# cordum-io/cordum

Hardware: AMD Instinct MI355X
Metric: jobs dispatched/sec (whole node) (higher is better)
Workload: dtype int64-bitset/int32 (control-plane integer path); 1 GPU; model=cordum control-plane dispatch pipeline (echo workers), global_batch=16384, seq_len=256, parallelism=shard1, rules=1024, workers_per_rank=1000, denied_jobs=14465

## Files before the change

cordum_amd/ops/hip/cordum_kernels.hip:

```cpp
#include <hip/hip_runtime.h>
#include <cstdint>

#define WAVE 64
#define BLOCK 256


template <int W, int JPT>
__global__ __launch_bounds__(BLOCK) void policy_first_match_kernel(
    const long long* __restrict__ rule_any,
    const long long* __restrict__ rule_all,
    const signed char* __restrict__ rule_secrets,
    const long long* __restrict__ rule_mcp,
    const unsigned char* __restrict__ rule_mcp_any,
    const long long* __restrict__ job_any,
    const long long* __restrict__ job_all,
    const unsigned char* __restrict__ job_secrets,
    const long long* __restrict__ job_mcp,
    const unsigned char* __restrict__ job_mcp_used,
    int* __restrict__ out_first,
    int R, int J, int rules_per_chunk)
{
    const int rule_chunk_begin = blockIdx.y * rules_per_chunk;
    const int rule_chunk_end = min(R, rule_chunk_begin + rules_per_chunk);
    constexpr int ANY_W = 7 * W;
// ... 1657 lines not shown
__global__ __launch_bounds__(BLOCK) void policy_first_match_mfma_bits_kernel(
    const long long* __restrict__ any_bits,
    const long long* __restrict__ all_bits,
    const signed char* __restrict__ b_pack,
    const int* __restrict__ cards,
    const signed char* __restrict__ rule_secrets,
    const unsigned char* __restrict__ job_secrets,
    const int* __restrict__ tile_dims,
    int* __restrict__ out_first,
    int J, int R, int tiles_per_chunk)
{
    const int lane = threadIdx.x % WAVE;
    const int shift = (lane >> 4) * 16;
    v4i afrag[TJ][9];
    #pragma unroll
    for (int t = 0; t < TJ; ++t) {
        const int job = (blockIdx.x * TJ + t) * 16 + (lane & 15);
        #pragma unroll
        for (int d = 0; d < 9; ++d) {
            unsigned long long w = 0;
            if (job < J)
                w = (unsigned long long)(d < 7 ? any_bits[(size_t)job * 7 + d]
                                               : all_bits[(size_t)job * 2 + (d - 7)]);
            const unsigned int slice = (unsigned int)(w >> shift) & 0xFFFFu;
            #pragma unroll
            for (int q = 0; q < 4; ++q)
                afrag[t][d][q] = (int)((((slice >> (4 * q)) & 0xFu) * 0x00204081u) & 0x01010101u);
        }
    }
    mfma_first_match_tiles<TJ>(afrag, b_pack, cards, rule_secrets, job_secrets,
                               tile_dims, out_first, J, R, tiles_per_chunk);
}


__global__ __launch_bounds__(BLOCK) void policy_gate_kernel(
    const int* __restrict__ first,
    const signed char* __restrict__ decisions,
    signed char* __restrict__ out_decision,
    int* __restrict__ denied_slots,
    int* __restrict__ denied_count,
    int* __restrict__ allowed_slots,
    int* __restrict__ allowed_count,
    int J, int R)
{
    const int j = blockIdx.x * BLOCK + threadIdx.x;
    const int lane = threadIdx.x % WAVE;
    gate_job(j, J, lane, first, decisions, R, out_decision,
             allowed_slots, allowed_count, denied_slots, denied_count);
}

__global__ __launch_bounds__(BLOCK) void policy_gate_full_kernel(
    const int* __restrict__ first,
    const signed char* __restrict__ decisions,
    signed char* __restrict__ out_decision,
    int* __restrict__ denied_slots,
    int* __restrict__ denied_count,
    int* __restrict__ allowed_slots,
    int* __restrict__ allowed_count,
    unsigned char* __restrict__ states,
    long long* __restrict__ deadlines,
    int* __restrict__ dlq_ring,
    int* __restrict__ dlq_head,
    int ring_size,
    int J, int R)
{
    const int j = blockIdx.x * BLOCK + threadIdx.x;
// ... 894 lines not shown
    torch::Tensor tile_dims, int64_t n_rules, torch::Tensor out, int64_t job_tiles)
{
    CHECK_DEV(any_bits); CHECK_DEV(b_pack);
    CHECK_CONTIG(any_bits); CHECK_CONTIG(all_bits);
    TORCH_CHECK(job_tiles == 1 || job_tiles == 2, "job_tiles must be 1 or 2");
    TORCH_CHECK(any_bits.dim() == 3 && any_bits.size(1) == 7 && any_bits.size(2) == 1 &&
                all_bits.dim() == 3 && all_bits.size(1) == 2 && all_bits.size(2) == 1,
                "MFMA K1 needs the 1-word vocab: any [J,7,1], all [J,2,1]");
    const int J = (int)any_bits.size(0), R = (int)n_rules;
    TORCH_CHECK(all_bits.size(0) == J && job_secrets.size(0) >= J && out.size(0) >= J,
                "job tensors must cover J");
    const int TJ = (int)job_tiles;
    const int Jt = ((J + 15) / 16 + TJ - 1) / TJ;
    const int Rt = (R + 15) / 16;
    if (J == 0 || R == 0) return;
    TORCH_CHECK(b_pack.size(0) >= Rt && tile_dims.size(0) >= Rt &&
                rule_secrets.size(0) >= Rt * 16 && cards.size(0) >= Rt * 16,
                "rule pack smaller than n_rules");
    int nchunks = std::max(1, std::min((Rt + 3) / 4, std::max(1, 2048 / std::max(Jt, 1))));
    const int tiles_per_chunk = (Rt + nchunks - 1) / nchunks;
    auto launch = [&](auto kernel) {
        hipLaunchKernelGGL(kernel, dim3(Jt, nchunks), dim3(BLOCK), 0, cur_stream(),
            (const long long*)any_bits.data_ptr<int64_t>(),
            (const long long*)all_bits.data_ptr<int64_t>(),
            (const signed char*)b_pack.data_ptr<int8_t>(),
            cards.data_ptr<int>(),
            (const signed char*)rule_secrets.data_ptr<int8_t>(),
            job_secrets.data_ptr<uint8_t>(),
            tile_dims.data_ptr<int>(),
            out.data_ptr<int>(), J, R, tiles_per_chunk);
    };
    if (TJ == 2) launch(policy_first_match_mfma_bits_kernel<2>);
    else launch(policy_first_match_mfma_bits_kernel<1>);
}

void gate_route(torch::Tensor first, torch::Tensor decisions, torch::Tensor out_decision,
                torch::Tensor denied_slots, torch::Tensor denied_count,
                torch::Tensor allowed_slots, torch::Tensor allowed_count,
                torch::Tensor states, torch::Tensor deadlines,
                torch::Tensor dlq_ring, torch::Tensor dlq_head,
                torch::Tensor pick, torch::Tensor order, torch::Tensor valid_count,
                torch::Tensor j_poolmask, torch::Tensor j_labels,
                int64_t full_mask, int64_t K,
                torch::Tensor routable_slots, torch::Tensor routable_widx,
                torch::Tensor routable_count, torch::Tensor extra_zero)
{
    CHECK_DEV(first);
    const int J = (int)first.size(0);
    TORCH_CHECK(out_decision.size(0) >= J && denied_slots.size(0) >= J &&
                allowed_slots.size(0) >= J && states.size(0) >= J &&
                deadlines.size(0) >= J && pick.size(0) >= J &&
                j_poolmask.size(0) >= J && j_labels.size(0) >= J &&
                routable_slots.size(0) >= J && routable_widx.size(0) >= J,
                "per-job tensors must cover J");
    TORCH_CHECK(K <= order.size(0), "K exceeds the order table");
    const int n_extra = (int)extra_zero.size(0);
    const int blocks = (std::max(std::max(J, n_extra), 1) + BLOCK - 1) / BLOCK;
    hipLaunchKernelGGL(gate_route_kernel, dim3(blocks), dim3(BLOCK), 0, cur_stream(),
        first.data_ptr<int>(), (const signed char*)decisions.data_ptr<int8_t>(),
        (signed char*)out_decision.data_ptr<int8_t>(),
        denied_slots.data_ptr<int>(), denied_count.data_ptr<int>(),
        allowed_slots.data_ptr<int>(), allowed_count.data_ptr<int>(),
        states.data_ptr<uint8_t>(), (long long*)deadlines.data_ptr<int64_t>(),
        dlq_ring.data_ptr<int>(), dlq_head.data_ptr<int>(), (int)dlq_ring.size(0),
        pick.data_ptr<int>(), order.data_ptr<int>(), valid_count.data_ptr<int>(),
        (const long long*)j_poolmask.data_ptr<int64_t>(),
// ... 660 lines not shown
                             int64_t all_requires,
                             c10::optional<torch::Tensor> payload,
                             int64_t payload_words,
                             int64_t threads, int64_t isa_cap)
{
    TORCH_CHECK(!any_bits.is_cuda() && !all_bits.is_cuda(),
                "synthetic_fresh_stamped is a host encoder");
    CHECK_CONTIG(any_bits); CHECK_CONTIG(all_bits);
    CHECK_CONTIG(tenant_lut); CHECK_CONTIG(topic_lut);
    CHECK_CONTIG(risk_lut); CHECK_CONTIG(req_lut);
    cordum_enc::EncodeJob a;
    a.B = any_bits.size(0);
    a.W = any_bits.size(2);
    a.V = tenant_lut.size(0);
    TORCH_CHECK(any_bits.size(1) == 7 && all_bits.size(0) == a.B &&
                all_bits.size(1) == 2 && all_bits.size(2) == a.W, "bad batch shape");
    for (const torch::Tensor* l : {&tenant_lut, &topic_lut, &risk_lut, &req_lut})
        TORCH_CHECK(l->size(0) == a.V && l->size(1) == a.W, "bad LUT shape");
    TORCH_CHECK(dim_tenant >= 0 && dim_tenant < 7 && dim_topic >= 0 && dim_topic < 7 &&
                dim_risk >= 0 && dim_risk < 7 && all_requires >= 0 && all_requires < 2,
                "dim index out of range");
    a.any = any_bits.data_ptr<int64_t>();
    a.all = all_bits.data_ptr<int64_t>();
    a.tenant_lut = tenant_lut.data_ptr<int64_t>();
    a.topic_lut = topic_lut.data_ptr<int64_t>();
    a.risk_lut = risk_lut.data_ptr<int64_t>();
    a.req_lut = req_lut.data_ptr<int64_t>();
    a.seed = (uint64_t)seed;
    a.step = (uint64_t)step;
    a.dim_tenant = (int)dim_tenant;
    a.dim_topic = (int)dim_topic;
    a.dim_risk = (int)dim_risk;
    a.all_requires = (int)all_requires;
    a.payload = nullptr;
    a.payload_words = payload_words;
    if (payload.has_value()) {
        TORCH_CHECK(!payload->is_cuda() && payload->is_contiguous() &&
                    payload->scalar_type() == torch::kInt32 && payload_words > 0 &&
                    payload->numel() >= a.B * payload_words, "bad payload ring buffer");
        a.payload = payload->data_ptr<int32_t>();
    }
    cordum_enc::encode_batch(a, (int)threads, (int)isa_cap);
}

void pack_jobs_mfma_dev(torch::Tensor any_bits, torch::Tensor all_bits,
                        torch::Tensor a_pack)
{
    const int B = (int)any_bits.size(0);
    const int Jt = (int)a_pack.size(0);
    const int n = Jt * 9 * 64;
    const int blocks = (n + BLOCK - 1) / BLOCK;
    hipLaunchKernelGGL(pack_jobs_mfma_kernel, dim3(blocks), dim3(BLOCK), 0, cur_stream(),
        (const long long*)any_bits.data_ptr<int64_t>(),
        (const long long*)all_bits.data_ptr<int64_t>(),
        a_pack.data_ptr<int8_t>(), B, Jt);
}

PYBIND11_MODULE(TORCH_EXTENSION_NAME, m) {
    m.def("policy_first_match", &policy_first_match, "K1 batched policy first-match");
    m.def("policy_first_match_mfma", &policy_first_match_mfma, "K1 MFMA comparison variant");
    m.def("worker_precompute", &worker_precompute, "K2a per-worker score/overload precompute");
    m.def("least_loaded_pick", &least_loaded_pick, "K2 least-loaded worker pick");
    m.def("spread_pick", &spread_pick, "K2c batch spreading over the least-loaded set");
    m.def("worker_precompute_into", &worker_precompute_into, "K2a into a persistent key tensor");
    m.def("dlq_ring_append", &dlq_ring_append, "K7 device DLQ ring append");
    m.def("echo_execute_indexed", &echo_execute_indexed, "device echo worker pool (slot-indexed, in-place)");
    m.def("policy_gate", &policy_gate, "decision gather + allow/deny compaction");
    m.def("policy_gate_full", &policy_gate_full,
          "gate + DENIED transition + DLQ ring append in one launch");
    m.def("begin_tick", &begin_tick, "tick prologue: PENDING re-admit + counter reset");
    m.def("accumulate_counts", &accumulate_counts, "fold tick counters into device accumulator");
    m.def("begin_tick_first", &begin_tick_first,
          "tick prologue that also primes the first-match buffer (INT_MAX)");
    m.def("least_loaded_pick_into", &least_loaded_pick_into,
          "K2 pick into a persistent buffer, skipping unconstrained jobs");
    m.def("policy_first_match_mfma_into", &policy_first_match_mfma_into,
          "K1 MFMA into a pre-primed buffer (no alloc/fill launches)");
    m.def("compact_routable_spread", &compact_routable_spread,
          "routable compaction with inline K2c spread");
    m.def("apply_transitions_chain_dyn", &apply_transitions_chain_dyn,
          "K5 chained targets in one launch (+ extra zero region)");
    m.def("compact_routable", &compact_routable, "routable-slot compaction");
    m.def("apply_transitions_dyn", &apply_transitions_dyn, "K5 with device-resident count");
    m.def("echo_execute_indexed_dyn", &echo_execute_indexed_dyn, "echo worker with device count");
    m.def("load_feedback", &load_feedback, "per-worker active-count histogram");
    m.def("run_readiness", &run_readiness, "K3 run/step readiness sweep");
    m.def("synthetic_fresh", &synthetic_fresh,
          py::call_guard<py::gil_scoped_release>(),
          "fused host synthetic-batch encoder");
    m.def("pack_jobs_mfma_dev", &pack_jobs_mfma_dev, "device job packing for the MFMA K1");
    m.def("synthetic_fresh_stamped", &synthetic_fresh_stamped,
          py::call_guard<py::gil_scoped_release>(),
          "host batch preparation in one call: synthetic dims + payload step stamp",
          py::arg("any_bits"), py::arg("all_bits"), py::arg("tenant_lut"),
          py::arg("topic_lut"), py::arg("risk_lut"), py::arg("req_lut"),
          py::arg("seed"), py::arg("step"), py::arg("dim_tenant"), py::arg("dim_topic"),
          py::arg("dim_risk"), py::arg("all_requires"), py::arg("payload"),
          py::arg("payload_words"), py::arg("threads") = 1, py::arg("isa_cap") = -1);
    m.def("encoder_isa_level", [] { return cordum_enc::max_isa_level(); },
          "widest encoder ISA this CPU runs (0 baseline, 1 AVX2, 2 AVX-512DQ)");
    m.def("tick_prologue", &tick_prologue,
          "fused tick 1/5: PENDING re-admit + counter reset + first prime + worker keys");
    m.def("policy_first_match_mfma_bits_into", &policy_first_match_mfma_bits_into,
          "fused tick 3/5: K1 MFMA with A fragments built from the staged bit words",
          py::arg("any_bits"), py::arg("all_bits"), py::arg("b_pack"), py::arg("cards"),
          py::arg("rule_secrets"), py::arg("job_secrets"), py::arg("tile_dims"),
          py::arg("n_rules"), py::arg("out"), py::arg("job_tiles") = 1);
    m.def("gate_route", &gate_route,
          "fused tick 4/5: gate + DENIED/DLQ + spread/exact pick + routable compaction");
    m.def("tick_finish", &tick_finish,
          "fused tick 5/5: echo + state chain + load feedback + counter fold");
    m.def("pack_by_dest", &pack_by_dest, "padded per-destination dispatch pack");
    m.def("pack_requeue", &pack_requeue, "redeliver last tick's requeue ring into the send segments");
    m.def("wf_sweep", &wf_sweep, "K3-WF readiness sweep + approval holds + condition/delay commits");
    m.def("wf_expand", &wf_expand, "K3-WF for_each/worker child expansion into the child arena");
    m.def("wf_apply", &wf_apply, "K3-WF child result application with failure injection");
    m.def("wf_apply_dead", &wf_apply_dead, "K3-WF dead-letter child application");
    m.def("wf_commit", &wf_commit, "K3-WF step aggregation + retry/backoff commit");
    m.def("wf_timeout_scan", &wf_timeout_scan, "K4-WF stale-step timeout scan");
    m.def("wf_readmit", &wf_readmit, "K3-WF continuous run re-admission from template");
    m.def("wf_status", &wf_status, "K3-WF run status roll-up");
    m.def("wf_grant", &wf_grant, "K3-WF host approval grants");
    m.def("wf_admit", &wf_admit, "K3-WF run admission into the lowest free slots");
    m.def("wf_cancel", &wf_cancel, "K3-WF generation-checked run cancellation");
    m.def("wf_retire", &wf_retire, "K3-WF completion records + quiescent slot release");
    m.def("wf_journal", &wf_journal, "K3-WF step-transition journal pass (observer)");
    m.def("wf_hold_scan", &wf_hold_scan, "K3-WF approval hold scan (open / expire / close holds)");
    m.def("wf_settle", &wf_settle, "K3-WF per-step-policy timeout + commit pass (replaces the scan/commit pair)");
    m.def("wf_hold_list", &wf_hold_list, "K3-WF ordered page of open approval holds");
    m.def("wf_decide", &wf_decide, "K3-WF generation-checked approval decisions");
    m.def("materialize_rq_payload", &materialize_rq_payload, "copy requeued payload rows into the rq arena");
    m.def("gather_payload_padded", &gather_payload_padded, "payload gather into padded send arena");
    m.def("echo_padded", &echo_padded, "region-valid echo over padded recv arena");
    m.def("apply_transitions_padded", &apply_transitions_padded, "K5 over padded slot list");
    m.def("load_feedback_padded", &load_feedback_padded, "padded per-worker load histogram");
    m.def("set_transition_lut", &set_transition_lut, "upload transition legality LUT");
    m.def("apply_transitions", &apply_transitions, "K5 batched state transitions");
    m.def("deadline_scan", &deadline_scan, "K4 deadline/staleness scan");
// ... 3 lines not shown
```

cordum_amd/ops/hip/synthetic_encode.h:

```cpp
#pragma once

#include <cstddef>
#include <cstdint>
#include <thread>

namespace cordum_enc {

struct EncodeJob {
    int64_t* any;
    int64_t* all;
    const int64_t* tenant_lut;
    const int64_t* topic_lut;
    const int64_t* risk_lut;
    const int64_t* req_lut;
    int64_t B, W, V;
    uint64_t seed, step;
    int dim_tenant, dim_topic, dim_risk, all_requires;
    int32_t* payload;
    int64_t payload_words;
};

constexpr int kBlock = 64;
constexpr uint32_t kRiskCut = 1288490189u;
constexpr uint32_t kReqCut = 429496730u;

static inline uint64_t splitmix64(uint64_t x) {
    x += 0x9E3779B97F4A7C15ull;
    x = (x ^ (x >> 30)) * 0xBF58476D1CE4E5B9ull;
    x = (x ^ (x >> 27)) * 0x94D049BB133111EBull;
    return x ^ (x >> 31);
}

static inline uint64_t batch_base(uint64_t seed, uint64_t step) {
    return splitmix64(seed * 0x5851F42D4C957F2Dull ^ step);
}

__attribute__((always_inline)) static inline void encode_range_impl(
    const EncodeJob& a, int64_t i0, int64_t i1)
{
    const uint64_t base = batch_base(a.seed, a.step);
    const uint64_t v = (uint64_t)a.V;
    const int64_t W = a.W;
    const int32_t stamp = (int32_t)(uint32_t)a.step;
    uint32_t t_idx[kBlock], o_idx[kBlock], r_idx[kBlock], q_idx[kBlock];
    uint32_t c_risk[kBlock], c_req[kBlock];
    for (int64_t b0 = i0; b0 < i1; b0 += kBlock) {
        const int n = (int)((i1 - b0) < kBlock ? (i1 - b0) : kBlock);
        for (int k = 0; k < kBlock; ++k) {
            const uint64_t h0 = splitmix64(base ^ (uint64_t)(b0 + k));
            const uint64_t h1 = splitmix64(h0);
            const uint64_t h2 = splitmix64(h1);
            t_idx[k] = (uint32_t)(((h0 & 0xffffffffull) * v) >> 32);
            o_idx[k] = (uint32_t)(((h0 >> 32) * v) >> 32);
            r_idx[k] = (uint32_t)(((h1 & 0xffffffffull) * v) >> 32);
            q_idx[k] = (uint32_t)(((h1 >> 32) * v) >> 32);
            c_risk[k] = (uint32_t)h2;
            c_req[k] = (uint32_t)(h2 >> 32);
        }
        if (W == 1) {
            int64_t* arow = a.any + (size_t)b0 * 7;
            int64_t* lrow = a.all + (size_t)b0 * 2;
            for (int k = 0; k < n; ++k, arow += 7, lrow += 2) {
                arow[a.dim_tenant] = a.tenant_lut[t_idx[k]];
                arow[a.dim_topic] = a.topic_lut[o_idx[k]];
                arow[a.dim_risk] = c_risk[k] < kRiskCut ? a.risk_lut[r_idx[k]] : 0;
                lrow[a.all_requires] = c_req[k] < kReqCut ? a.req_lut[q_idx[k]] : 0;
            }
        } else {
            for (int k = 0; k < n; ++k) {
                int64_t* arow = a.any + (size_t)(b0 + k) * 7 * W;
                int64_t* lrow = a.all + (size_t)(b0 + k) * 2 * W;
                const bool has_risk = c_risk[k] < kRiskCut;
                const bool has_req = c_req[k] < kReqCut;
                const int64_t* tl = a.tenant_lut + (size_t)t_idx[k] * W;
                const int64_t* ol = a.topic_lut + (size_t)o_idx[k] * W;
                const int64_t* rl = a.risk_lut + (size_t)r_idx[k] * W;
                const int64_t* ql = a.req_lut + (size_t)q_idx[k] * W;
                for (int64_t w = 0; w < W; ++w) {
                    arow[a.dim_tenant * W + w] = tl[w];
                    arow[a.dim_topic * W + w] = ol[w];
                    arow[a.dim_risk * W + w] = has_risk ? rl[w] : 0;
                    lrow[a.all_requires * W + w] = has_req ? ql[w] : 0;
                }
            }
        }
        if (a.payload != nullptr) {
            int32_t* p = a.payload + (size_t)b0 * a.payload_words;
            for (int k = 0; k < n; ++k, p += a.payload_words) *p = stamp;
        }
    }
}

static void encode_range_base(const EncodeJob& a, int64_t i0, int64_t i1) {
    encode_range_impl(a, i0, i1);
}

#if defined(__x86_64__) && (defined(__GNUC__) || defined(__clang__)) && \
    !defined(__HIP_DEVICE_COMPILE__)
#define CORDUM_ENC_MULTIVERSION 1
__attribute__((target("avx2"))) static void encode_range_avx2(
    const EncodeJob& a, int64_t i0, int64_t i1) {
    encode_range_impl(a, i0, i1);
}
__attribute__((target("avx512f,avx512dq,avx512vl"))) static void encode_range_avx512(
    const EncodeJob& a, int64_t i0, int64_t i1) {
    encode_range_impl(a, i0, i1);
}
static inline int max_isa_level() {
    __builtin_cpu_init();
    if (__builtin_cpu_supports("avx512f") && __builtin_cpu_supports("avx512dq") &&
        __builtin_cpu_supports("avx512vl"))
        return 2;
    if (__builtin_cpu_supports("avx2")) return 1;
    return 0;
}
// ... 29 lines not shown
```

cordum_amd/ops/pipeline.py:

```python
from __future__ import annotations

import time
from dataclasses import dataclass
from typing import List, Optional

import torch
import torch.distributed as dist

from ..protocol.states import transition_lut
from ..safety import policy as pol
from . import get_ext
from .policy_compile import CompiledPolicy, JobBatch, JobEncoder, compile_policy, first_match_reference

UNSPECIFIED, PENDING, APPROVAL, SCHEDULED, DISPATCHED, RUNNING = 0, 1, 2, 3, 4, 5
SUCCEEDED, FAILED, CANCELLED, TIMEOUT, DENIED = 6, 7, 8, 9, 10

ALLOW_CODES = (1, 5)


@dataclass
class TickStats:
    completed: int = 0
    denied: int = 0
    unrouted: int = 0
# ... 102 lines not shown
        out.any_bits[:, DIM_TOPIC].copy_(row)
        torch.index_select(self.risk_lut, 0, r_idx, out=row)
        mask.view(-1).copy_(u_risk < 0.3)
        row.mul_(mask)
        out.any_bits[:, DIM_RISK].copy_(row)
        torch.index_select(self.req_lut, 0, q_idx, out=row)
        mask.view(-1).copy_(u_req < 0.1)
        row.mul_(mask)
        out.all_bits[:, ALL_REQUIRES].copy_(row)

    def fresh_fast(self, out: JobBatch, step: int, ext) -> None:
        DIM_TENANT, DIM_TOPIC, DIM_RISK, ALL_REQUIRES = self._dims
        ext.synthetic_fresh(out.any_bits, out.all_bits,
                            self.tenant_lut, self.topic_lut,
                            self.risk_lut, self.req_lut,
                            self.seed, step,
                            DIM_TENANT, DIM_TOPIC, DIM_RISK, ALL_REQUIRES)

    encode_threads = 1

    def fresh_stamped(self, out: JobBatch, step: int, ext, payload: torch.Tensor,
                      payload_words: int, threads: Optional[int] = None,
                      isa_cap: int = -1) -> None:
        DIM_TENANT, DIM_TOPIC, DIM_RISK, ALL_REQUIRES = self._dims
        ext.synthetic_fresh_stamped(out.any_bits, out.all_bits,
                                    self.tenant_lut, self.topic_lut,
                                    self.risk_lut, self.req_lut,
                                    self.seed, step,
                                    DIM_TENANT, DIM_TOPIC, DIM_RISK, ALL_REQUIRES,
                                    payload, payload_words,
                                    self.encode_threads if threads is None else threads,
                                    isa_cap)


class _RefOps:

    def __init__(self):
        self._lut = None

    def set_transition_lut(self, lut):
        self._lut = lut

    def policy_first_match(self, rule_any, rule_all, rule_secrets, rule_mcp, rule_mcp_any,
                           job_any, job_all, job_secrets, job_mcp, job_mcp_used, chunks):
        from types import SimpleNamespace

        c = SimpleNamespace(any_masks=rule_any, all_masks=rule_all, secrets=rule_secrets,
                            mcp_masks=rule_mcp, mcp_any=rule_mcp_any,
                            n_rules=int(rule_any.shape[0]))
        b = SimpleNamespace(any_bits=job_any, all_bits=job_all, secrets=job_secrets,
                            mcp_bits=job_mcp, mcp_used=job_mcp_used,
                            n_jobs=int(job_any.shape[0]))
        return first_match_reference(c, b)

    def worker_precompute(self, w_pool, w_active, w_maxp, w_cpu, w_gpu):
        from .reference import worker_precompute_ref

        return worker_precompute_ref(w_pool, w_active, w_maxp, w_cpu, w_gpu)

    def least_loaded_pick(self, w_pool, w_keys, w_labels, j_poolmask, j_labels):
        from .reference import least_loaded_pick_keys_ref

        return least_loaded_pick_keys_ref(w_pool, w_keys, w_labels, j_poolmask, j_labels)

    def echo_execute_indexed(self, ctx_arena, slots, res_arena, res_sum, stride):
        from .reference import echo_execute_indexed_ref
# ... 275 lines not shown
        return apply_transitions_ref(states, attempts, deadlines, slots, to_states)

    def echo_execute(self, ctx_arena, res_arena, stride):
        from .reference import echo_execute_ref

        return echo_execute_ref(ctx_arena, res_arena, int(stride))


def alloc_batch_staging(B: int, W: int, device=None, pin: bool = False):
    n64 = B * 7 * W + B * 2 * W + B * 4 * W
    nbytes = ((n64 * 8 + 2 * B + 7) // 8) * 8
    if pin:
        buf = torch.zeros(nbytes, dtype=torch.uint8).pin_memory()
    else:
        buf = torch.zeros(nbytes, dtype=torch.uint8, device=device)
    o = 0

    def take64(*shape):
        nonlocal o
        n = 1
        for s in shape:
            n *= s
        t = buf[o:o + n * 8].view(torch.int64).view(*shape)
        o += n * 8
        return t

    any_b = take64(B, 7, W)
    all_b = take64(B, 2, W)
    mcp_b = take64(B, 4, W)
    sec = buf[o:o + B]
    o += B
    used = buf[o:o + B]
    return JobBatch(any_b, all_b, sec, mcp_b, used), buf


def alloc_result_block(B: int, device=None, pin: bool = False):
    nbytes = ((4 * B + 16 + B + 7) // 8) * 8
    if pin:
        buf = torch.zeros(nbytes, dtype=torch.uint8).pin_memory()
    else:
        buf = torch.zeros(nbytes, dtype=torch.uint8, device=device)
    sums = buf[0:4 * B].view(torch.int32)
    counts = buf[4 * B:4 * B + 16].view(torch.int32)
    dec = buf[4 * B + 16:5 * B + 16].view(torch.int8)
    return sums, counts, dec, buf


class DevicePipeline:
    def __init__(
        self,
        device: torch.device,
        batch_size: int = 16384,
        n_local_workers: int = 1000,
        n_rules: int = 1024,
        payload_words: int = 64,
        world_size: int = 1,
        rank: int = 0,
        n_batches: int = 8,
        policy: Optional[pol.SafetyPolicy] = None,
        seed: int = 7,
        backend: str = "ext",
        use_mfma: Optional[bool] = None,
        mfma_pack_on_device: bool = False,
        pad_cap: Optional[int] = None,
        unfused_tick: bool = False,
        k1_job_tiles: int = 2,
    ):
        self._k1_job_tiles = k1_job_tiles
        self._pad_cap_override = pad_cap
        self._unfused_tick = unfused_tick
        self._mfma_device_pack = mfma_pack_on_device
        device = torch.device(device)
        self.ext = _RefOps() if backend == "ref" else get_ext(required=True)
        self.device = device
        self.B = batch_size
        self.NWL = n_local_workers
        self.world = world_size
        self.rank = rank
        self.payload_words = payload_words

        self.ext.set_transition_lut(torch.tensor(transition_lut(), dtype=torch.uint8).flatten())

        policy = policy or make_synthetic_policy(n_rules, seed=seed)
        for w in (1, 2, 4):
            self.compiled = compile_policy(policy, words=w)
            if self.compiled.exact:
                break
        assert self.compiled.exact, "bench policy must compile exactly"
        self.cpol = self.compiled.to(device)

        self.batches: List[JobBatch] = []
        self.batch_bufs: List[torch.Tensor] = []
        self.payloads: List[torch.Tensor] = []
        for i in range(n_batches):
            jb = encode_synthetic_jobs(self.compiled, self.B, seed=seed * 1000 + i + rank * 77)
            dev_jb, dev_buf = alloc_batch_staging(self.B, self.compiled.words,
                                                  device=device)
            dev_jb.any_bits.copy_(jb.any_bits)
            dev_jb.all_bits.copy_(jb.all_bits)
# ... 60 lines not shown
            backend != "ref"
            and device.type == "cuda"
            and world_size == 1
            and self.compiled.words == 1
            and self.compiled.n_rules <= 32768
            and int(self.compiled.mcp_any.sum()) == 0
        )
        if use_mfma is False:
            self._use_mfma = False
        if self._use_mfma and self._mfma_device_pack:
            from .policy_mfma import N_DIMS, pack_policy_mfma

            self.mfma_policy = pack_policy_mfma(self.compiled).to(device)
            self.mfma_a_packs = []
            if self._unfused_tick:
                Jt = (self.B + 15) // 16
                self.mfma_a_packs = [
                    torch.zeros(Jt, N_DIMS, 64, 16, dtype=torch.int8, device=device)
                    for _ in range(len(self.batches))
                ]
        elif self._use_mfma:
            from .policy_mfma import pack_jobs_mfma, pack_policy_mfma

            self.mfma_policy = pack_policy_mfma(self.compiled).to(device)
            self.mfma_a_packs = []
            for jb_host, jb_dev in zip(
                [encode_synthetic_jobs(self.compiled, self.B, seed=seed * 1000 + i + rank * 77)
                 for i in range(len(self.batches) if self._unfused_tick else 0)],
                self.batches
            ):
                a_pack, _ = pack_jobs_mfma(jb_host)
                self.mfma_a_packs.append(a_pack.to(device))
        self._fused_capable = device.type == "cuda" and self.world == 1 and backend != "ref"
        self._tick = 0
        self.total_completed = 0
        self.total_denied = 0


    def _spread(self, pick):
        full_mask = (1 << self.world) - 1
        K = min(int(self.order_buf.shape[0]), 1024)
        self.ext.spread_pick(self.order_buf, self.valid_buf, self.j_poolmask,
                             self.j_labels, full_mask, pick, K)
        return pick

    def _refresh_order(self) -> None:
        if self._tick % 8 != 1:
            return
        self.order_buf.copy_(torch.argsort(self.w_keys).to(torch.int32))
        valid = ((self.w_keys >> 32) & 0xFFFFFFFF).ne(0xFFFFFFFE)
        self.valid_buf.copy_(valid.sum().to(torch.int32).reshape(1))

    def _fused_body(self, slot: int) -> None:
        if self._unfused_tick:
            return self._unfused_body(slot)
        B = self.B
        ext = self.ext
        jb = self.batches[slot]
        full_mask = (1 << self.world) - 1
        ext.tick_prologue(self.states, self._counts,
                          self.first_buf if self._use_mfma else None,
                          self.w_active_local, self.w_maxp,
                          self.w_cpu_local, self.w_gpu_local, self.w_keys)
        ext.least_loaded_pick_into(self.w_pool, self.w_keys, self.w_labels,
                                   self.j_poolmask, self.j_labels,
                                   self.valid_buf, full_mask, self.pick_buf)
        if self._use_mfma:
            ext.policy_first_match_mfma_bits_into(
                jb.any_bits, jb.all_bits, self.mfma_policy.b_pack,
                self.mfma_policy.cards, self.mfma_policy.secrets, jb.secrets,
                self.mfma_policy.tile_dims, self.compiled.n_rules, self.first_buf,
                self._k1_job_tiles)
            first = self.first_buf
        else:
            first = ext.policy_first_match(
                self.cpol.any_masks, self.cpol.all_masks, self.cpol.secrets,
                self.cpol.mcp_masks, self.cpol.mcp_any,
                jb.any_bits, jb.all_bits, jb.secrets, jb.mcp_bits, jb.mcp_used, 0,
            )
        K = min(int(self.order_buf.shape[0]), 1024)
        ext.gate_route(first, self.cpol.decisions, self.out_decision,
                       self.denied_slots, self.denied_count,
                       self.allowed_slots, self.allowed_count,
                       self.states, self.deadlines, self.dlq_ring, self.dlq_head,
                       self.pick_buf, self.order_buf, self.valid_buf,
                       self.j_poolmask, self.j_labels, full_mask, K,
                       self.routable_slots, self.routable_widx,
                       self.routable_count, self.w_active_local)
        ext.tick_finish(self.payloads[slot], self.routable_slots,
                        self.routable_widx, self.routable_count,
                        self.res_arena[: B * self.payload_words], self.res_sums,
                        self.payload_words,
                        self.states, self.attempts, self.deadlines,
                        [SCHEDULED, DISPATCHED, RUNNING, SUCCEEDED],
                        self.w_active_local, self.NWL, self.rank,
                        self._counts, self.acc_counts, B)

    def _unfused_body(self, slot: int) -> None:
        B = self.B
        ext = self.ext
# ... 36 lines not shown
                                    self.routable_count)
        ext.echo_execute_indexed_dyn(self.payloads[slot], self.routable_slots,
                                     self.routable_count, self.res_arena[: B * self.payload_words],
                                     self.res_sums, self.payload_words, B)
        ext.apply_transitions_chain_dyn(self.states, self.attempts, self.deadlines,
                                        self.routable_slots, self.routable_count,
                                        [SCHEDULED, DISPATCHED, RUNNING, SUCCEEDED],
                                        self.w_active_local, B)
        ext.load_feedback(self.routable_widx, self.routable_count,
                          self.w_active_local, self.NWL, self.rank, B)
        ext.accumulate_counts(self._counts, self.acc_counts)

    def _ensure_graphs(self) -> None:
        if self._graphs:
            return
        side = torch.cuda.Stream(device=self.device)
        side.wait_stream(torch.cuda.current_stream(self.device))
        with torch.cuda.stream(side):
            for slot in range(len(self.batches)):
                self._fused_body(slot)
        torch.cuda.current_stream(self.device).wait_stream(side)
        torch.cuda.synchronize(self.device)
        for slot in range(len(self.batches)):
            g = torch.cuda.CUDAGraph()
            with torch.cuda.graph(g):
                self._fused_body(slot)
            self._graphs[slot] = g
        self._graph = self._graphs[0]
        self.dlq_head.zero_()
        self.dlq_ring.fill_(-1)
        self.acc_counts.zero_()
        torch.cuda.synchronize(self.device)

    def _replay_fused(self) -> None:
        i = self._tick % len(self.batches)
        self._tick += 1
        self._graphs[i].replay()
        self._refresh_order()

    def _tick_fused(self) -> TickStats:
        self._ensure_graphs()
        t0 = time.perf_counter()
        self._replay_fused()
        counts = self._counts.cpu()
        denied = int(counts[0])
        routable = int(counts[2])
        dt = time.perf_counter() - t0
        stats = TickStats(
            completed=routable,
            denied=denied,
            unrouted=self.B - routable - denied,
            wall_s=dt,
        )
        self.total_completed += stats.completed
        self.total_denied += stats.denied
        return stats

    def ensure_e2e(self, seed: int = 11, payload_ring: int = 4) -> None:
        if hasattr(self, "_e2e_enc"):
            return
        assert not self._use_mfma or self._mfma_device_pack, \
            "e2e ingest needs staged descriptors: bitset K1 or device-packed MFMA"
        self._e2e_enc = SyntheticEncoder(self.compiled, seed=seed + self.rank)
        pin = self.device.type == "cuda"
        B, W = self.B, self.compiled.words

# ... 109 lines not shown
            return self._e2e_run_dist(steps)
        if self.device.type != "cuda" or not self._fused_capable:
            completed = denied = 0
            lats = []
            for _ in range(steps):
                st = self.tick_e2e()
                completed += st.completed
                denied += st.denied
                lats.append(st.wall_s)
            return completed, denied, lats

        self._ensure_graphs()
        B = self.B
        nslots = 2
        nhost = 4
        if not hasattr(self, "_e2e_hosts2"):
            Wc = self.compiled.words
            pairs = [alloc_batch_staging(B, Wc, pin=True) for _ in range(nhost)]
            self._e2e_hosts2 = [p[0] for p in pairs]
            self._e2e_host_bufs = [p[1] for p in pairs]
            self._e2e_encs = [SyntheticEncoder(self.compiled, seed=101 + 13 * i + self.rank)
                              for i in range(nhost)]
            outs = [alloc_result_block(B, pin=True) for _ in range(nslots)]
            self._e2e_out_sums = [o[0] for o in outs]
            self._e2e_out_counts = [o[1] for o in outs]
            self._e2e_out_dec = [o[2] for o in outs]
            self._e2e_out_blocks = [o[3] for o in outs]
            self._e2e_ev = [torch.cuda.Event() for _ in range(nslots)]
            self._e2e_in_ev = [torch.cuda.Event() for _ in range(nslots)]
            self._e2e_copy_stream = torch.cuda.Stream(device=self.device)
            from concurrent.futures import ThreadPoolExecutor

            self._e2e_pool = ThreadPoolExecutor(max_workers=2)

        completed = denied = 0
        lats = [0.0] * steps
        t_enc = [0.0] * steps

        def encode(s: int):
            t_enc[s] = time.perf_counter()
            self._encode_host(s, self._e2e_hosts2[s % nhost], self._e2e_encs[s % nhost],
                              self._e2e_payloads[s % len(self._e2e_payloads)])

        def harvest(s_prev: int) -> None:
            nonlocal completed, denied
            slot = s_prev % nslots
            self._e2e_ev[slot].synchronize()
            c = self._e2e_out_counts[slot]
            denied_n = int(c[0])
            routable = int(c[2])
            completed += routable
            denied += denied_n
            lats[s_prev] = time.perf_counter() - t_enc[s_prev]
            self._e2e_sums = self._e2e_out_sums[slot]
            self._e2e_decisions = self._e2e_out_dec[slot]

        futs = {}

        def submit(s: int) -> None:
            if s < steps:
                futs[s] = self._e2e_pool.submit(encode, s)

        submit(0)
        submit(1)
        for s in range(steps):
            futs.pop(s).result()
            slot = s % nslots
            with torch.cuda.stream(self._e2e_copy_stream):
                self.batch_bufs[slot].copy_(
                    self._e2e_host_bufs[s % nhost], non_blocking=True)
                self.payloads[slot].copy_(
                    self._e2e_payloads[s % len(self._e2e_payloads)],
                    non_blocking=True)
                self._e2e_in_ev[slot].record(self._e2e_copy_stream)
            torch.cuda.current_stream(self.device).wait_event(self._e2e_in_ev[slot])
            self._graphs[slot].replay()
            self._e2e_out_blocks[slot].copy_(self._res_block, non_blocking=True)
            self._e2e_ev[slot].record()
            submit(s + 2)
            if s >= 1:
                harvest(s - 1)
        harvest(steps - 1)
        return completed, denied, lats

    def tick(self) -> TickStats:
        if getattr(self, "_fused_capable", False):
            return self._tick_fused()
        if self.world > 1:
            return self._tick_padded()
        return self._tick_eager()

    def reset_stats(self) -> None:
        self.acc_counts.zero_()
        self.total_completed = 0
        self.total_denied = 0

    def tick_async(self) -> None:
        if getattr(self, "_fused_capable", False):
            self._ensure_graphs()
            self._replay_fused()
            return
        if self.world > 1 and self.device.type == "cuda":
            self._pad_alloc()
            self._ensure_pad_graphs()
            self._run_padded()
            return
        st = self.tick()
        if self.world == 1:
            self.acc_counts[0] += st.denied
# ... 360 lines not shown
```

cordum_amd/ops/policy_mfma.py:

```python
from __future__ import annotations

from dataclasses import dataclass
from typing import Tuple

import torch

from .policy_compile import CompiledPolicy, JobBatch

N_DIMS = 9
VOCAB = 64


def _bits_to_onehot(words: torch.Tensor) -> torch.Tensor:
    n, d, w = words.shape
    assert w == 1, "MFMA variant supports 1-word (vocab<=64) policies"
    shifts = torch.arange(64, dtype=torch.int64)
    return ((words >> shifts.view(1, 1, 64)) & 1).to(torch.int8)


def _pack_a(onehot: torch.Tensor) -> torch.Tensor:
    J = onehot.shape[0]
    Jt = (J + 15) // 16
    padded = torch.zeros(Jt * 16, N_DIMS, VOCAB, dtype=torch.int8)
    padded[:J] = onehot
    a = padded.view(Jt, 16, N_DIMS, 4, 16)
    a = a.permute(0, 2, 3, 1, 4).reshape(Jt, N_DIMS, 64, 16)
    return a.contiguous()


def _pack_b(onehot: torch.Tensor) -> torch.Tensor:
    R = onehot.shape[0]
    Rt = (R + 15) // 16
    padded = torch.zeros(Rt * 16, N_DIMS, VOCAB, dtype=torch.int8)
    padded[:R] = onehot
    b = padded.view(Rt, 16, N_DIMS, 4, 16)
    b = b.permute(0, 2, 3, 1, 4)
    b = b.reshape(Rt, N_DIMS, 64, 16)
    return b.contiguous()


@dataclass
class MfmaPolicy:
    b_pack: torch.Tensor
    cards: torch.Tensor
    secrets: torch.Tensor
    tile_dims: torch.Tensor
    n_rules: int

    def to(self, device):
        return MfmaPolicy(self.b_pack.to(device), self.cards.to(device),
                          self.secrets.to(device), self.tile_dims.to(device),
                          self.n_rules)


def pack_policy_mfma(c: CompiledPolicy) -> MfmaPolicy:
    assert c.words == 1, "MFMA variant needs vocab <= 64"
    R = c.n_rules
    rule_bits = torch.cat([c.any_masks, c.all_masks], dim=1)
    onehot = _bits_to_onehot(rule_bits)
    b_pack = _pack_b(onehot)
    Rt = b_pack.shape[0]
    cards = torch.zeros(Rt * 16, N_DIMS, dtype=torch.int32)
    cards[:R] = onehot.sum(dim=2).to(torch.int32)
    if Rt * 16 > R:
        cards[R:, 7] = 127
    secrets = torch.full((Rt * 16,), -1, dtype=torch.int8)
    secrets[:R] = c.secrets
    used = (cards.view(Rt, 16, N_DIMS) != 0).any(dim=1)
    tile_dims = (used.to(torch.int32) << torch.arange(N_DIMS, dtype=torch.int32)).sum(
        dim=1).to(torch.int32)
    return MfmaPolicy(b_pack, cards, secrets, tile_dims, R)


def pack_jobs_mfma(jobs: JobBatch) -> Tuple[torch.Tensor, torch.Tensor]:
    job_bits = torch.cat([jobs.any_bits, jobs.all_bits], dim=1)
    onehot = _bits_to_onehot(job_bits)
    return _pack_a(onehot), jobs.secrets


def first_match_mfma(ext, mp: MfmaPolicy, a_pack: torch.Tensor,
                     job_secrets: torch.Tensor, n_jobs: int) -> torch.Tensor:
    return ext.policy_first_match_mfma(
        a_pack, mp.b_pack, mp.cards, mp.secrets, job_secrets, mp.tile_dims,
        int(n_jobs), int(mp.n_rules),
    )
```

Measured before the change: 117.6 million jobs/s.

## Stage only policy-live dimension columns for host encode, H2D copy and K1

Adds a compact staging layout that keeps only the job bitset dimensions some rule actually reads (derived from tile_dims), with a col_map telling the MFMA K1 kernel which column backs each dimension. The host encoder writes straight into these compact rows, the end-to-end loop copies the smaller pinned buffer to the device, and separate CUDA graphs use a new cols-based K1. The aim is to shrink host encode work and the H2D transfer per batch, and it is on by default when the fused MFMA tick is available. In exchange it adds a second graph set and a host-side tile_dims check outside capture, and it relies on the live-dim map staying in step with the packed policy.

Measured after the change: 129.6 million jobs/s, median of 6. 10.3% higher.

```diff
diff --git a/cordum_amd/ops/hip/cordum_kernels.hip b/cordum_amd/ops/hip/cordum_kernels.hip
--- a/cordum_amd/ops/hip/cordum_kernels.hip
+++ b/cordum_amd/ops/hip/cordum_kernels.hip
@@ -1713,6 +1713,40 @@
                                tile_dims, out_first, J, R, tiles_per_chunk);
 }
 
+template <int TJ>
+__global__ __launch_bounds__(BLOCK) void policy_first_match_mfma_cols_kernel(
+    const long long* __restrict__ cols,
+    int L, unsigned long long col_map,
+    const signed char* __restrict__ b_pack,
+    const int* __restrict__ cards,
+    const signed char* __restrict__ rule_secrets,
+    const unsigned char* __restrict__ job_secrets,
+    const int* __restrict__ tile_dims,
+    int* __restrict__ out_first,
+    int J, int R, int tiles_per_chunk)
+{
+    const int lane = threadIdx.x % WAVE;
+    const int shift = (lane >> 4) * 16;
+    v4i afrag[TJ][9];
+    #pragma unroll
+    for (int t = 0; t < TJ; ++t) {
+        const int job = (blockIdx.x * TJ + t) * 16 + (lane & 15);
+        #pragma unroll
+        for (int d = 0; d < 9; ++d) {
+            const int c = (int)((col_map >> (4 * d)) & 0xFull);
+            unsigned long long w = 0;
+            if (c < L && job < J)
+                w = (unsigned long long)cols[(size_t)job * L + c];
+            const unsigned int slice = (unsigned int)(w >> shift) & 0xFFFFu;
+            #pragma unroll
+            for (int q = 0; q < 4; ++q)
+                afrag[t][d][q] = (int)((((slice >> (4 * q)) & 0xFu) * 0x00204081u) & 0x01010101u);
+        }
+    }
+    mfma_first_match_tiles<TJ>(afrag, b_pack, cards, rule_secrets, job_secrets,
+                               tile_dims, out_first, J, R, tiles_per_chunk);
+}
+
 
 __global__ __launch_bounds__(BLOCK) void policy_gate_kernel(
     const int* __restrict__ first,
@@ -2673,6 +2707,65 @@
     };
     if (TJ == 2) launch(policy_first_match_mfma_bits_kernel<2>);
     else launch(policy_first_match_mfma_bits_kernel<1>);
+}
+
+void policy_first_match_mfma_cols_into(
+    torch::Tensor cols, int64_t col_map,
+    torch::Tensor b_pack, torch::Tensor cards,
+    torch::Tensor rule_secrets, torch::Tensor job_secrets,
+    torch::Tensor tile_dims, int64_t n_rules, torch::Tensor out, int64_t job_tiles)
+{
+    CHECK_DEV(cols); CHECK_DEV(b_pack);
+    CHECK_CONTIG(cols);
+    TORCH_CHECK(job_tiles == 1 || job_tiles == 2, "job_tiles must be 1 or 2");
+    TORCH_CHECK(cols.dim() == 2 && cols.scalar_type() == torch::kInt64 && cols.size(1) <= 9,
+                "compact K1 needs cols [J,L] int64 with L <= 9 (1-word vocab)");
+    const int J = (int)cols.size(0), R = (int)n_rules, L = (int)cols.size(1);
+    TORCH_CHECK(job_secrets.size(0) >= J && out.size(0) >= J, "job tensors must cover J");
+    TORCH_CHECK(col_map >= 0 && (col_map >> 36) == 0, "col_map holds 9 nibbles");
+    unsigned map_dims = 0;
+    int next_col = 0;
+    for (int d = 0; d < 9; ++d) {
+        const int c = (int)((col_map >> (4 * d)) & 0xF);
+        if (c == 0xF) continue;
+        TORCH_CHECK(c == next_col, "col_map must number the live dims 0..L-1 in ascending d");
+        ++next_col;
+        map_dims |= 1u << d;
+    }
+    TORCH_CHECK(next_col == L, "col_map names ", next_col, " columns, cols has ", L);
+    const int TJ = (int)job_tiles;
+    const int Jt = ((J + 15) / 16 + TJ - 1) / TJ;
+    const int Rt = (R + 15) / 16;
+    if (J == 0 || R == 0) return;
+    TORCH_CHECK(b_pack.size(0) >= Rt && tile_dims.size(0) >= Rt &&
+                rule_secrets.size(0) >= Rt * 16 && cards.size(0) >= Rt * 16,
+                "rule pack smaller than n_rules");
+    hipStreamCaptureStatus capturing = hipStreamCaptureStatusNone;
+    TORCH_CHECK(hipStreamIsCapturing(cur_stream(), &capturing) == hipSuccess,
+                "hipStreamIsCapturing failed");
+    if (capturing == hipStreamCaptureStatusNone) {
+        const torch::Tensor td = tile_dims.narrow(0, 0, Rt).cpu();
+        const int* p = td.data_ptr<int>();
+        unsigned scanned = 0;
+        for (int rt = 0; rt < Rt; ++rt) scanned |= (unsigned)p[rt];
+        TORCH_CHECK((scanned & 0x1FFu & ~map_dims) == 0,
+                    "col_map lacks a dimension the packed policy scans (stale map?): "
+                    "tile_dims union ", scanned & 0x1FFu, ", map dims ", map_dims);
+    }
+    int nchunks = std::max(1, std::min((Rt + 3) / 4, std::max(1, 2048 / std::max(Jt, 1))));
+    const int tiles_per_chunk = (Rt + nchunks - 1) / nchunks;
+    auto launch = [&](auto kernel) {
+        hipLaunchKernelGGL(kernel, dim3(Jt, nchunks), dim3(BLOCK), 0, cur_stream(),
+            (const long long*)cols.data_ptr<int64_t>(), L, (unsigned long long)col_map,
+            (const signed char*)b_pack.data_ptr<int8_t>(),
+            cards.data_ptr<int>(),
+            (const signed char*)rule_secrets.data_ptr<int8_t>(),
+            job_secrets.data_ptr<uint8_t>(),
+            tile_dims.data_ptr<int>(),
+            out.data_ptr<int>(), J, R, tiles_per_chunk);
+    };
+    if (TJ == 2) launch(policy_first_match_mfma_cols_kernel<2>);
+    else launch(policy_first_match_mfma_cols_kernel<1>);
 }
 
 void gate_route(torch::Tensor first, torch::Tensor decisions, torch::Tensor out_decision,
@@ -3399,6 +3492,59 @@
     a.dim_topic = (int)dim_topic;
     a.dim_risk = (int)dim_risk;
     a.all_requires = (int)all_requires;
+    a.payload = nullptr;
+    a.payload_words = payload_words;
+    if (payload.has_value()) {
+        TORCH_CHECK(!payload->is_cuda() && payload->is_contiguous() &&
+                    payload->scalar_type() == torch::kInt32 && payload_words > 0 &&
+                    payload->numel() >= a.B * payload_words, "bad payload ring buffer");
+        a.payload = payload->data_ptr<int32_t>();
+    }
+    cordum_enc::encode_batch(a, (int)threads, (int)isa_cap);
+}
+
+void synthetic_fresh_compact(torch::Tensor cols,
+                             torch::Tensor tenant_lut, torch::Tensor topic_lut,
+                             torch::Tensor risk_lut, torch::Tensor req_lut,
+                             int64_t seed, int64_t step,
+                             int64_t col_of_tenant, int64_t col_of_topic,
+                             int64_t col_of_risk, int64_t col_of_requires,
+                             c10::optional<torch::Tensor> payload,
+                             int64_t payload_words,
+                             int64_t threads, int64_t isa_cap)
+{
+    TORCH_CHECK(!cols.is_cuda(), "synthetic_fresh_compact is a host encoder");
+    CHECK_CONTIG(cols);
+    CHECK_CONTIG(tenant_lut); CHECK_CONTIG(topic_lut);
+    CHECK_CONTIG(risk_lut); CHECK_CONTIG(req_lut);
+    TORCH_CHECK(cols.dim() == 2 && cols.scalar_type() == torch::kInt64,
+                "cols must be [B,L] int64");
+    cordum_enc::EncodeJob a;
+    a.B = cols.size(0);
+    a.W = 1;
+    a.V = tenant_lut.size(0);
+    const int64_t L = cols.size(1);
+    for (const torch::Tensor* l : {&tenant_lut, &topic_lut, &risk_lut, &req_lut})
+        TORCH_CHECK(l->dim() == 2 && l->size(0) == a.V && l->size(1) == 1,
+                    "compact rows need 1-word LUTs [V,1]");
+    const int64_t c4[4] = {col_of_tenant, col_of_topic, col_of_risk, col_of_requires};
+    for (int i = 0; i < 4; ++i) {
+        TORCH_CHECK(c4[i] >= -1 && c4[i] < L, "column index out of range");
+        for (int k = 0; k < i; ++k)
+            TORCH_CHECK(c4[i] < 0 || c4[i] != c4[k], "two dims share a column");
+    }
+    a.any = a.all = cols.data_ptr<int64_t>();
+    a.any_stride = a.all_stride = L;
+    a.tenant_lut = tenant_lut.data_ptr<int64_t>();
+    a.topic_lut = topic_lut.data_ptr<int64_t>();
+    a.risk_lut = risk_lut.data_ptr<int64_t>();
+    a.req_lut = req_lut.data_ptr<int64_t>();
+    a.seed = (uint64_t)seed;
+    a.step = (uint64_t)step;
+    a.dim_tenant = (int)col_of_tenant;
+    a.dim_topic = (int)col_of_topic;
+    a.dim_risk = (int)col_of_risk;
+    a.all_requires = (int)col_of_requires;
     a.payload = nullptr;
     a.payload_words = payload_words;
     if (payload.has_value()) {
@@ -3464,6 +3610,14 @@
           py::arg("seed"), py::arg("step"), py::arg("dim_tenant"), py::arg("dim_topic"),
           py::arg("dim_risk"), py::arg("all_requires"), py::arg("payload"),
           py::arg("payload_words"), py::arg("threads") = 1, py::arg("isa_cap") = -1);
+    m.def("synthetic_fresh_compact", &synthetic_fresh_compact,
+          py::call_guard<py::gil_scoped_release>(),
+          "synthetic_fresh_stamped into compact rows: one column per dim the policy reads",
+          py::arg("cols"), py::arg("tenant_lut"), py::arg("topic_lut"),
+          py::arg("risk_lut"), py::arg("req_lut"), py::arg("seed"), py::arg("step"),
+          py::arg("col_of_tenant"), py::arg("col_of_topic"), py::arg("col_of_risk"),
+          py::arg("col_of_requires"), py::arg("payload"), py::arg("payload_words"),
+          py::arg("threads") = 1, py::arg("isa_cap") = -1);
     m.def("encoder_isa_level", [] { return cordum_enc::max_isa_level(); },
           "widest encoder ISA this CPU runs (0 baseline, 1 AVX2, 2 AVX-512DQ)");
     m.def("tick_prologue", &tick_prologue,
@@ -3471,6 +3625,12 @@
     m.def("policy_first_match_mfma_bits_into", &policy_first_match_mfma_bits_into,
           "fused tick 3/5: K1 MFMA with A fragments built from the staged bit words",
           py::arg("any_bits"), py::arg("all_bits"), py::arg("b_pack"), py::arg("cards"),
+          py::arg("rule_secrets"), py::arg("job_secrets"), py::arg("tile_dims"),
+          py::arg("n_rules"), py::arg("out"), py::arg("job_tiles") = 1);
+    m.def("policy_first_match_mfma_cols_into", &policy_first_match_mfma_cols_into,
+          "fused tick 3/5, compact staging: K1 MFMA with A fragments built from the "
+          "live-dimension columns",
+          py::arg("cols"), py::arg("col_map"), py::arg("b_pack"), py::arg("cards"),
           py::arg("rule_secrets"), py::arg("job_secrets"), py::arg("tile_dims"),
           py::arg("n_rules"), py::arg("out"), py::arg("job_tiles") = 1);
     m.def("gate_route", &gate_route,
diff --git a/cordum_amd/ops/hip/synthetic_encode.h b/cordum_amd/ops/hip/synthetic_encode.h
--- a/cordum_amd/ops/hip/synthetic_encode.h
+++ b/cordum_amd/ops/hip/synthetic_encode.h
@@ -18,6 +18,8 @@
     int dim_tenant, dim_topic, dim_risk, all_requires;
     int32_t* payload;
     int64_t payload_words;
+    int64_t any_stride = 0;
+    int64_t all_stride = 0;
 };
 
 constexpr int kBlock = 64;
@@ -41,6 +43,10 @@
     const uint64_t base = batch_base(a.seed, a.step);
     const uint64_t v = (uint64_t)a.V;
     const int64_t W = a.W;
+    const int64_t sa = a.any_stride > 0 ? a.any_stride : 7;
+    const int64_t sl = a.all_stride > 0 ? a.all_stride : 2;
+    const bool st = a.dim_tenant >= 0, so = a.dim_topic >= 0;
+    const bool sr = a.dim_risk >= 0, sq = a.all_requires >= 0;
     const int32_t stamp = (int32_t)(uint32_t)a.step;
     uint32_t t_idx[kBlock], o_idx[kBlock], r_idx[kBlock], q_idx[kBlock];
     uint32_t c_risk[kBlock], c_req[kBlock];
@@ -57,19 +63,20 @@
             c_risk[k] = (uint32_t)h2;
             c_req[k] = (uint32_t)(h2 >> 32);
         }
-        if (W == 1) {
-            int64_t* arow = a.any + (size_t)b0 * 7;
-            int64_t* lrow = a.all + (size_t)b0 * 2;
-            for (int k = 0; k < n; ++k, arow += 7, lrow += 2) {
-                arow[a.dim_tenant] = a.tenant_lut[t_idx[k]];
-                arow[a.dim_topic] = a.topic_lut[o_idx[k]];
-                arow[a.dim_risk] = c_risk[k] < kRiskCut ? a.risk_lut[r_idx[k]] : 0;
-                lrow[a.all_requires] = c_req[k] < kReqCut ? a.req_lut[q_idx[k]] : 0;
+        if (!(st || so || sr || sq)) {
+        } else if (W == 1) {
+            int64_t* arow = a.any + (size_t)b0 * sa;
+            int64_t* lrow = a.all + (size_t)b0 * sl;
+            for (int k = 0; k < n; ++k, arow += sa, lrow += sl) {
+                if (st) arow[a.dim_tenant] = a.tenant_lut[t_idx[k]];
+                if (so) arow[a.dim_topic] = a.topic_lut[o_idx[k]];
+                if (sr) arow[a.dim_risk] = c_risk[k] < kRiskCut ? a.risk_lut[r_idx[k]] : 0;
+                if (sq) lrow[a.all_requires] = c_req[k] < kReqCut ? a.req_lut[q_idx[k]] : 0;
             }
         } else {
             for (int k = 0; k < n; ++k) {
-                int64_t* arow = a.any + (size_t)(b0 + k) * 7 * W;
-                int64_t* lrow = a.all + (size_t)(b0 + k) * 2 * W;
+                int64_t* arow = a.any + (size_t)(b0 + k) * sa * W;
+                int64_t* lrow = a.all + (size_t)(b0 + k) * sl * W;
                 const bool has_risk = c_risk[k] < kRiskCut;
                 const bool has_req = c_req[k] < kReqCut;
                 const int64_t* tl = a.tenant_lut + (size_t)t_idx[k] * W;
@@ -77,10 +84,10 @@
                 const int64_t* rl = a.risk_lut + (size_t)r_idx[k] * W;
                 const int64_t* ql = a.req_lut + (size_t)q_idx[k] * W;
                 for (int64_t w = 0; w < W; ++w) {
-                    arow[a.dim_tenant * W + w] = tl[w];
-                    arow[a.dim_topic * W + w] = ol[w];
-                    arow[a.dim_risk * W + w] = has_risk ? rl[w] : 0;
-                    lrow[a.all_requires * W + w] = has_req ? ql[w] : 0;
+                    if (st) arow[a.dim_tenant * W + w] = tl[w];
+                    if (so) arow[a.dim_topic * W + w] = ol[w];
+                    if (sr) arow[a.dim_risk * W + w] = has_risk ? rl[w] : 0;
+                    if (sq) lrow[a.all_requires * W + w] = has_req ? ql[w] : 0;
                 }
             }
         }
diff --git a/cordum_amd/ops/pipeline.py b/cordum_amd/ops/pipeline.py
--- a/cordum_amd/ops/pipeline.py
+++ b/cordum_amd/ops/pipeline.py
@@ -158,6 +158,25 @@
                                     self.encode_threads if threads is None else threads,
                                     isa_cap)
 
+    def compact_columns(self, live) -> tuple:
+        from .policy_mfma import col_of
+
+        DIM_TENANT, DIM_TOPIC, DIM_RISK, ALL_REQUIRES = self._dims
+        return (col_of(live, DIM_TENANT), col_of(live, DIM_TOPIC),
+                col_of(live, DIM_RISK), col_of(live, 7 + ALL_REQUIRES))
+
+    def fresh_compact(self, cols: torch.Tensor, step: int, ext, columns,
+                      payload: torch.Tensor, payload_words: int,
+                      threads: Optional[int] = None, isa_cap: int = -1) -> None:
+        assert self.W == 1, "compact rows need the 1-word vocab"
+        ct, co, cr, cq = columns
+        ext.synthetic_fresh_compact(cols, self.tenant_lut, self.topic_lut,
+                                    self.risk_lut, self.req_lut,
+                                    self.seed, step, ct, co, cr, cq,
+                                    payload, payload_words,
+                                    self.encode_threads if threads is None else threads,
+                                    isa_cap)
+
 
 class _RefOps:
 
@@ -499,6 +518,18 @@
     o += B
     used = buf[o:o + B]
     return JobBatch(any_b, all_b, sec, mcp_b, used), buf
+
+
+def alloc_compact_staging(B: int, L: int, device=None, pin: bool = False):
+    assert B >= 1 and 0 <= L <= 9
+    nbytes = ((B * L * 8 + B + 7) // 8) * 8
+    if pin:
+        buf = torch.zeros(nbytes, dtype=torch.uint8).pin_memory()
+    else:
+        buf = torch.zeros(nbytes, dtype=torch.uint8, device=device)
+    cols = buf[0:B * L * 8].view(torch.int64).view(B, L)
+    sec = buf[B * L * 8:B * L * 8 + B]
+    return cols, sec, buf
 
 
 def alloc_result_block(B: int, device=None, pin: bool = False):
@@ -532,6 +563,7 @@
         pad_cap: Optional[int] = None,
         unfused_tick: bool = False,
         k1_job_tiles: int = 2,
+        compact_staging: Optional[bool] = None,
     ):
         self._k1_job_tiles = k1_job_tiles
         self._pad_cap_override = pad_cap
@@ -658,9 +690,39 @@
                 a_pack, _ = pack_jobs_mfma(jb_host)
                 self.mfma_a_packs.append(a_pack.to(device))
         self._fused_capable = device.type == "cuda" and self.world == 1 and backend != "ref"
+        compact_ok = (self._fused_capable and self._use_mfma
+                      and self._mfma_device_pack and not self._unfused_tick)
+        if compact_staging and not compact_ok:
+            raise ValueError("compact_staging needs the fused MFMA-from-bits tick "
+                             "(single rank, 1-word vocabulary, CUDA, ext backend, "
+                             "mfma_pack_on_device)")
+        self._compact = compact_ok if compact_staging is None else bool(compact_staging)
+        if self._compact:
+            self._build_compact()
         self._tick = 0
         self.total_completed = 0
         self.total_denied = 0
+
+    def _build_compact(self) -> None:
+        from .policy_mfma import col_map, gather_live_cols, live_dims
+
+        self._live = live_dims(self.mfma_policy)
+        self._col_map = col_map(self._live)
+        self.compact_cols: List[torch.Tensor] = []
+        self.compact_secrets: List[torch.Tensor] = []
+        self.compact_bufs: List[torch.Tensor] = []
+        for jb in self.batches:
+            cols, sec, buf = alloc_compact_staging(self.B, len(self._live),
+                                                   device=self.device)
+            cols.copy_(gather_live_cols(jb, self._live))
+            sec.copy_(jb.secrets)
+            self.compact_cols.append(cols)
+            self.compact_secrets.append(sec)
+            self.compact_bufs.append(buf)
+        self._cgraphs = {}
+        for name in ("_e2e_ccols", "_e2e_cbufs", "_e2e_ccolumns"):
+            if hasattr(self, name):
+                delattr(self, name)
 
 
     def _spread(self, pick):
@@ -677,7 +739,8 @@
         valid = ((self.w_keys >> 32) & 0xFFFFFFFF).ne(0xFFFFFFFE)
         self.valid_buf.copy_(valid.sum().to(torch.int32).reshape(1))
 
-    def _fused_body(self, slot: int) -> None:
+    def _fused_body(self, slot: int, compact: bool = False) -> None:
+        assert not compact or self._compact, "compact staging is off"
         if self._unfused_tick:
             return self._unfused_body(slot)
         B = self.B
@@ -691,7 +754,14 @@
         ext.least_loaded_pick_into(self.w_pool, self.w_keys, self.w_labels,
                                    self.j_poolmask, self.j_labels,
                                    self.valid_buf, full_mask, self.pick_buf)
-        if self._use_mfma:
+        if compact:
+            ext.policy_first_match_mfma_cols_into(
+                self.compact_cols[slot], self._col_map, self.mfma_policy.b_pack,
+                self.mfma_policy.cards, self.mfma_policy.secrets,
+                self.compact_secrets[slot], self.mfma_policy.tile_dims,
+                self.compiled.n_rules, self.first_buf, self._k1_job_tiles)
+            first = self.first_buf
+        elif self._use_mfma:
             ext.policy_first_match_mfma_bits_into(
                 jb.any_bits, jb.all_bits, self.mfma_policy.b_pack,
                 self.mfma_policy.cards, self.mfma_policy.secrets, jb.secrets,
@@ -794,6 +864,28 @@
         self.acc_counts.zero_()
         torch.cuda.synchronize(self.device)
 
+    def _ensure_compact_graphs(self) -> None:
+        if self._cgraphs:
+            return
+        self._ensure_graphs()
+        keep = (self.dlq_head.clone(), self.dlq_ring.clone(), self.acc_counts.clone())
+        side = torch.cuda.Stream(device=self.device)
+        side.wait_stream(torch.cuda.current_stream(self.device))
+        with torch.cuda.stream(side):
+            for slot in range(len(self.batches)):
+                self._fused_body(slot, compact=True)
+        torch.cuda.current_stream(self.device).wait_stream(side)
+        torch.cuda.synchronize(self.device)
+        for slot in range(len(self.batches)):
+            g = torch.cuda.CUDAGraph()
+            with torch.cuda.graph(g):
+                self._fused_body(slot, compact=True)
+            self._cgraphs[slot] = g
+        self.dlq_head.copy_(keep[0])
+        self.dlq_ring.copy_(keep[1])
+        self.acc_counts.copy_(keep[2])
+        torch.cuda.synchronize(self.device)
+
     def _replay_fused(self) -> None:
         i = self._tick % len(self.batches)
         self._tick += 1
@@ -969,6 +1061,18 @@
             from concurrent.futures import ThreadPoolExecutor
 
             self._e2e_pool = ThreadPoolExecutor(max_workers=2)
+        compact = self._compact
+        if compact and not hasattr(self, "_e2e_cbufs"):
+            trip = [alloc_compact_staging(B, len(self._live), pin=True)
+                    for _ in range(nhost)]
+            self._e2e_ccols = [t[0] for t in trip]
+            self._e2e_cbufs = [t[2] for t in trip]
+            self._e2e_ccolumns = self._e2e_encs[0].compact_columns(self._live)
+        if compact:
+            self._ensure_compact_graphs()
+        graphs = self._cgraphs if compact else self._graphs
+        dev_bufs = self.compact_bufs if compact else self.batch_bufs
+        host_bufs = self._e2e_cbufs if compact else self._e2e_host_bufs
 
         completed = denied = 0
         lats = [0.0] * steps
@@ -976,8 +1080,14 @@
 
         def encode(s: int):
             t_enc[s] = time.perf_counter()
+            payload = self._e2e_payloads[s % len(self._e2e_payloads)]
+            if compact:
+                self._e2e_encs[s % nhost].fresh_compact(
+                    self._e2e_ccols[s % nhost], s, self.ext, self._e2e_ccolumns,
+                    payload, self.payload_words)
+                return
             self._encode_host(s, self._e2e_hosts2[s % nhost], self._e2e_encs[s % nhost],
-                              self._e2e_payloads[s % len(self._e2e_payloads)])
+                              payload)
 
         def harvest(s_prev: int) -> None:
             nonlocal completed, denied
@@ -1004,14 +1114,13 @@
             futs.pop(s).result()
             slot = s % nslots
             with torch.cuda.stream(self._e2e_copy_stream):
-                self.batch_bufs[slot].copy_(
-                    self._e2e_host_bufs[s % nhost], non_blocking=True)
+                dev_bufs[slot].copy_(host_bufs[s % nhost], non_blocking=True)
                 self.payloads[slot].copy_(
                     self._e2e_payloads[s % len(self._e2e_payloads)],
                     non_blocking=True)
                 self._e2e_in_ev[slot].record(self._e2e_copy_stream)
             torch.cuda.current_stream(self.device).wait_event(self._e2e_in_ev[slot])
-            self._graphs[slot].replay()
+            graphs[slot].replay()
             self._e2e_out_blocks[slot].copy_(self._res_block, non_blocking=True)
             self._e2e_ev[slot].record()
             submit(s + 2)
diff --git a/cordum_amd/ops/policy_mfma.py b/cordum_amd/ops/policy_mfma.py
--- a/cordum_amd/ops/policy_mfma.py
+++ b/cordum_amd/ops/policy_mfma.py
@@ -1,7 +1,7 @@
 from __future__ import annotations
 
 from dataclasses import dataclass
-from typing import Tuple
+from typing import List, Sequence, Tuple
 
 import torch
 
@@ -66,10 +66,43 @@
         cards[R:, 7] = 127
     secrets = torch.full((Rt * 16,), -1, dtype=torch.int8)
     secrets[:R] = c.secrets
-    used = (cards.view(Rt, 16, N_DIMS) != 0).any(dim=1)
+    real = torch.zeros(Rt * 16, N_DIMS, dtype=torch.bool)
+    real[:R] = cards[:R] != 0
+    used = real.view(Rt, 16, N_DIMS).any(dim=1)
     tile_dims = (used.to(torch.int32) << torch.arange(N_DIMS, dtype=torch.int32)).sum(
         dim=1).to(torch.int32)
     return MfmaPolicy(b_pack, cards, secrets, tile_dims, R)
+
+
+COL_ABSENT = 0xF
+
+
+def live_dims(mp: MfmaPolicy) -> List[int]:
+    union = 0
+    for v in mp.tile_dims.cpu().tolist():
+        union |= int(v)
+    return [d for d in range(N_DIMS) if (union >> d) & 1]
+
+
+def col_map(live: Sequence[int]) -> int:
+    live = list(live)
+    assert live == sorted(set(live)) and all(0 <= d < N_DIMS for d in live), live
+    m = 0
+    for d in range(N_DIMS):
+        m |= (live.index(d) if d in live else COL_ABSENT) << (4 * d)
+    return m
+
+
+def col_of(live: Sequence[int], d: int) -> int:
+    live = list(live)
+    return live.index(d) if d in live else -1
+
+
+def gather_live_cols(jobs: JobBatch, live: Sequence[int]) -> torch.Tensor:
+    assert jobs.any_bits.shape[2] == 1, "compact rows need the 1-word vocab"
+    job_bits = torch.cat([jobs.any_bits, jobs.all_bits], dim=1)[:, :, 0]
+    idx = torch.tensor(list(live), dtype=torch.int64, device=job_bits.device)
+    return job_bits.index_select(1, idx).contiguous()
 
 
 def pack_jobs_mfma(jobs: JobBatch) -> Tuple[torch.Tensor, torch.Tensor]:
```
